# Liaoyongjian1/HC-MVS

Hardware: AMD Instinct MI355X
Metric: PatchMatch Mpix/s (1080p, 8 views, 7x7, 8 iter) (higher is better)
Workload: dtype f32; 1 GPU; batch of 32 independent units per GPU, each 1 ref x 8 src views, 1920x1080, 7x7 taps (adapthalfwin 6), 8 sweeps, it_external 0, full EstimateDepthMap (median + init score + sweeps + end pass); batch=32, exchange=none

## Files before the change

hc-mvs_amd/csrc/est_plan.h:

```cpp
#ifndef HCMVS_EST_PLAN_H
#define HCMVS_EST_PLAN_H
#include <math.h>
#include <stddef.h>
#include <stdint.h>
#include <string.h>
#include "../../include/hcmvs_hip.h"
#include "carve.h"
#include "pm_types.h"
#include "sweep_plan.h"
namespace hcmvs {

inline float fd2r(float d) { return d * (3.14159274101257324f / 180.f); }

inline void mat3_mul(const double* a, const double* b, double* c) {
	for (int i = 0; i < 3; ++i)
		for (int j = 0; j < 3; ++j) {
			double s = 0;
			for (int k = 0; k < 3; ++k) s += a[i * 3 + k] * b[k * 3 + j];
			c[i * 3 + j] = s;
		}
}
inline void mat3_mul_bt(const double* a, const double* b, double* c) {
	for (int i = 0; i < 3; ++i)
		for (int j = 0; j < 3; ++j) {
// ... 94 lines not shown
	k.smoothBonusNormal = (1.f - p.random_smooth_bonus) * 0.96f;
	k.smoothSigmaDepth = -1.f / (2.f * (p.random_smooth_depth * p.random_smooth_depth));
	{ const float r = fd2r(p.random_smooth_normal_deg); k.smoothSigmaNormal = -1.f / (2.f * (r * r)); }
	k.angle1Range = fd2r(p.random_angle1_deg);
	k.angle2Range = fd2r(p.random_angle2_deg);
	k.thConfSmall = p.ncc_threshold_keep * 0.2f;
	k.thConfBig = p.ncc_threshold_keep * 0.4f;
	k.thConfRand = p.ncc_threshold_keep * 0.9f;
	k.thRobust = p.ncc_threshold_keep * 1.2f;
	k.thKeep = p.ncc_threshold_keep;
	k.depthRatio = p.random_depth_ratio;
	k.pfScale = 1.f - p.photometric_flow;
	k.seed = p.seed + seedOffset;
	k.hintIter = est_uses_hint(p, hintOffered) ? p.n_estimation_iters - 1 : -1;
}

inline bool est_view_spreads(bool viewspread, const hcmvs_params& p, bool offersMaps, bool rescaled) {
	return viewspread && p.it_external >= 1 && offersMaps && !rescaled;
}
inline void est_spread_consts(const EstCamera& ref, const EstCamera& s, SpreadView& sv) {
	sv.w = s.w; sv.h = s.h;
	sv.cx = s.K[2]; sv.cy = s.K[5]; sv.ifx = 1.0 / s.K[0]; sv.ify = 1.0 / s.K[4];
	double T[9];
	mat3_mul_bt(ref.R, s.R, T);
	const double dC[3] = {s.C[0] - ref.C[0], s.C[1] - ref.C[1], s.C[2] - ref.C[2]};
	sv.Tz[0] = T[6]; sv.Tz[1] = T[7]; sv.Tz[2] = T[8];
	sv.tz = ref.R[6] * dC[0] + ref.R[7] * dC[1] + ref.R[8] * dC[2];
}

inline SweepItem est_sweep_item(const EstConst& k, int nSweeps, bool prior = false, bool geo = false) {
	return {k.H - 2 * k.border, k.W - 2 * k.border, k.V, k.hintDepth && k.hintIter == nSweeps - 1, k.keep != nullptr, k.spread != nullptr, prior, geo};
}

constexpr uint64_t kEstWindowLimit = 0xFFFF0000ull;
enum EstWindowKind { kEstWindowDirect, kEstWindowSlab, kEstWindowRefused };
struct EstWindow {
	EstWindowKind kind;
	uint64_t base;
	size_t slabBytes;
};
inline EstWindow est_image_window(const uint64_t* addr, const size_t* bytes, int n, uint32_t* off) {
	uint64_t lo = ~(uint64_t)0, hi = 0;
	for (int v = 0; v < n; ++v) {
		if (addr[v] < lo) lo = addr[v];
		if (addr[v] + bytes[v] > hi) hi = addr[v] + bytes[v];
	}
	if (hi - lo < kEstWindowLimit) {
		for (int v = 0; v < n; ++v) off[v] = (uint32_t)(addr[v] - lo);
		return {kEstWindowDirect, lo, 0};
	}
	Carve slab;
	for (int v = 0; v < n; ++v) off[v] = (uint32_t)slab(bytes[v]);
	return {slab.size >= kEstWindowLimit ? kEstWindowRefused : kEstWindowSlab, 0, slab.size};
}

enum PriorBad { kPriorOk = 0, kPriorPara, kPriorSigma, kPriorPhoto2geo };
inline PriorBad est_check_prior_params(const hcmvs_prior_params& pp) {
	if (!(pp.para_prior >= 0.f && pp.para_prior <= 1.f)) return kPriorPara;
	if (!(pp.sigma_prior > 0.f) || !(pp.sigma_prior < INFINITY)) return kPriorSigma;
	if (pp.photo2geo < 0) return kPriorPhoto2geo;
	return kPriorOk;
}
inline bool est_prior_active(bool registered, const hcmvs_prior_params& pp, const hcmvs_params& p) {
	return registered && pp.para_prior > 0.f && p.it_external >= pp.photo2geo;
}
inline void est_prior_consts(const hcmvs_prior_params& pp, int countIter, PriorItem& k) {
// ... 107 lines not shown
```

hc-mvs_amd/csrc/hcmvs_api.cpp:

```cpp
#include "../../include/hcmvs_hip.h"
#include "pm_common.h"
#include "est_plan.h"
#include "fuse_common.h"
#include "pf_chain.h"
#include "filter_plan.h"
#include "fuse_plan.h"
#include "tri_init.h"
#include "cloud_kernels.h"
#include "vis_kernels.h"
#include "mesh_kernels.h"
#include "view_kernels.h"
#include "init_kernels.h"
#include "handoff_kernels.h"
#include "handoff_host.h"
#include "prior_kernels.h"
#include "dev_buf.h"

#include <cmath>
#include <cstdarg>
#include <cstdio>
#include <cstring>
#include <map>
#include <string>
#include <algorithm>
// ... 35 lines not shown

struct hcmvs_ctx final : Reclaimer {
	int device = 0;
	hipStream_t ownStream = nullptr;
	hipStream_t stream = nullptr;
	std::string err;
	std::map<uint32_t, View> views;
	struct Slot {
		explicit Slot(Reclaimer* r) : dn(r), conf(r), tmpDepth(r), progress(r), srcSlab(r) {}
		DevBuf dn, conf, tmpDepth;
		DevBuf progress;
		DevBuf srcSlab;
	};
	std::vector<Slot> slots;
	DevBuf tmpU8{this};
	DevBuf maskStage{this};
	DevBuf sDepth{this}, sNormal{this}, sConf{this};
	DevBuf dViews{this};
	std::vector<DevView> hViews;
	DevBuf dItems{this};
	std::vector<EstConst> hItems;
	DevBuf dSpread{this};
	std::vector<SpreadView> hSpread;
	int viewspread = 0;
	bool haveSpreadStats = false;
	hcmvs_prior_params prior = {0.5f, 0.2f, 2};
	bool havePriorStats = false;
	hcmvs_geo_params geo = {0, 0.25f, 0.15f, 150.f, 160.f, 2, 3.f};
	bool haveGeoStats = false;
	DevBuf dGeo{this};
	std::vector<GeoView> hGeo;
	DevBuf sync{this};
	SweepKnobs knobs;
	DevBuf evals{this};
	Event ev[4];
	int lastSweeps = 0, lastSweepLaunches = 0;
	bool haveStats = false;
	int fuseOrder = 0;
	DevBuf dMaps{this};
	DevBuf counters{this};
	DevBuf fuseScratch{this};
	DevBuf filterStage{this}, filterTab{this}, filterCnt{this};
	DevBuf passScratch{this};
	DevBuf pfState;
	bool errPending = false;
	int nCU = 0;
	PinnedBuf pinned;
	Event upEv[2] = {Event(hipEventDisableTiming), Event(hipEventDisableTiming)};
	DevBuf initBuf{this};
	PinnedBuf initPinned;
	Event initCopied{hipEventDisableTiming};
	bool initInFlight = false;
	Event initEv[2];
	hcmvs_init_stats initStats = {};
	bool haveInitStats = false;
	DevBuf handoffBuf{this};
	PinnedBuf handoffPinned;
	Event handoffEv[2];
	hcmvs_handoff_stats handoffStats = {};
	bool haveHandoffStats = false;
	DevBuf priorGenKept{this};
	PriorGenTrace priorTrace;

	bool reclaim() override {
		if (!pfState.capacity() && !priorGenKept.capacity()) return false;
		(void)hipStreamSynchronize(stream);
// ... 57 lines not shown
	p->random_smooth_bonus = 0.93f;
	p->photometric_flow = 0.f;
	p->seed = 1234;
	p->median_blur = 1;
}

int hcmvs_create(int device, hcmvs_ctx** out) {
	if (!out) return HCMVS_ERR_INVALID;
	*out = nullptr;
	int n = 0;
	if (hipGetDeviceCount(&n) != hipSuccess || n <= 0 || device < 0 || device >= n) return HCMVS_ERR_NO_DEVICE;
	if (hipSetDevice(device) != hipSuccess) return HCMVS_ERR_NO_DEVICE;
	hipDeviceProp_t prop;
	if (hipGetDeviceProperties(&prop, device) != hipSuccess) return HCMVS_ERR_NO_DEVICE;
	if (strncmp(prop.gcnArchName, "gfx950", 6) != 0) return HCMVS_ERR_NO_DEVICE;
	hcmvs_ctx* c = new hcmvs_ctx();
	c->device = device;
	c->nCU = prop.multiProcessorCount;
	if (hipStreamCreateWithFlags(&c->ownStream, hipStreamNonBlocking) != hipSuccess) { hcmvs_destroy(c); return HCMVS_ERR_NO_DEVICE; }
	c->stream = c->ownStream;
	for (Event& e : c->ev)
		if (e.ensure() != hipSuccess) { hcmvs_destroy(c); return HCMVS_ERR_NO_DEVICE; }
	c->hViews.resize((size_t)kMaxBatch * kViewSlotEntries); c->hItems.resize(kMaxBatch); c->hSpread.resize((size_t)kMaxBatch * kMaxViews);
	c->hGeo.resize((size_t)kMaxBatch * kMaxViews);
	if (c->dViews.reserve(sizeof(DevView) * kViewSlotEntries * kMaxBatch, c->stream) != hipSuccess || c->evals.reserve(128, c->stream) != hipSuccess ||
	    c->dSpread.reserve(sizeof(SpreadView) * kMaxViews * kMaxBatch, c->stream) != hipSuccess ||
	    c->dGeo.reserve(sizeof(GeoView) * kMaxViews * kMaxBatch, c->stream) != hipSuccess ||
	    c->dItems.reserve(sizeof(EstConst) * kMaxBatch, c->stream) != hipSuccess || c->sync.reserve(64 + sizeof(int32_t) * 2 * kMaxBatch, c->stream) != hipSuccess) {
		hcmvs_destroy(c);
		return HCMVS_ERR_NO_DEVICE;
	}
	c->knobs = parse_sweep_knobs(getenv("HCMVS_SWEEP_LAG"), getenv("HCMVS_XCD_AFFINITY"), getenv("HCMVS_SWEEP_LAUNCHES"), getenv("HCMVS_SWEEP_SEGMENT"),
	                             getenv("HCMVS_WAVES_PER_ROW"));
	*out = c;
	return HCMVS_OK;
}

void hcmvs_destroy(hcmvs_ctx* c) {
	if (!c) return;
	(void)hipSetDevice(c->device);
	(void)hipStreamSynchronize(c->stream);
	const hipStream_t own = c->ownStream;
	delete c;
	if (own) (void)hipStreamDestroy(own);
}

const char* hcmvs_last_error(const hcmvs_ctx* c) { return c ? c->err.c_str() : "null context"; }

static int check_sweep_error(hcmvs_ctx* c) {
	if (!c->errPending) return HCMVS_OK;
	int32_t flags[2] = {0, 0};
	HIPCHK(c, hipMemcpy(flags, c->sync.get(), sizeof flags, hipMemcpyDeviceToHost));
	c->errPending = false;
	if (flags[1] != 0) return fail(c, HCMVS_ERR_TIMEOUT, "sweep worker timed out waiting for its predecessor row; the maps of the last estimate are incomplete");
	return HCMVS_OK;
}

int hcmvs_set_stream(hcmvs_ctx* c, void* stream) {
	if (!c) return HCMVS_ERR_INVALID;
	c->stream = stream ? (hipStream_t)stream : c->ownStream;
	return HCMVS_OK;
}
int hcmvs_synchronize(hcmvs_ctx* c) {
	if (!c) return HCMVS_ERR_INVALID;
	HIPCHK(c, hipSetDevice(c->device));
	HIPCHK(c, hipStreamSynchronize(c->stream));
// ... 396 lines not shown
		batch.items.push_back(est_sweep_item(k, batch.nSweeps, itemPrior, itemGeo));
		maxRows = std::max(maxRows, batch.items.back().rows);
		spread = spread || k.spread;
		prior = prior || itemPrior;
		geo = geo || itemGeo;
	}
	if (spread) {
		const EstOverlap o = est_spread_overlap(c->hItems.data(), c->hSpread.data(), items, n_items);
		if (o.item >= 0)
			return fail(c, HCMVS_ERR_INVALID, "estimate: the in/out maps of item %d (view %u) overlap the spread maps of source view %u of item %d: "
			            "a launch must not read what it writes (register a copy, or estimate the two images in separate calls)", o.item, items[o.item].ref_id,
			            items[o.other].src_ids[o.view], o.other);
	}
	if (geo) {
		std::vector<char> act((size_t)n_items, 0);
		for (int i = 0; i < n_items; ++i) act[i] = batch.items[i].geo;
		const EstOverlap o = est_geo_overlap(c->hItems.data(), c->hGeo.data(), (const bool*)act.data(), items, n_items);
		if (o.item >= 0)
			return fail(c, HCMVS_ERR_INVALID, "estimate: the in/out maps of item %d (view %u) overlap the maps source view %u of item %d offers to the "
			            "geometric-consistency term: a launch must not read what it writes (register a copy, or estimate the two images in separate calls)",
			            o.item, items[o.item].ref_id, items[o.other].src_ids[o.view], o.other);
	}
	hipStream_t s = c->stream;
	if (geo) HIPCHK(c, hipMemcpyAsync(c->dGeo.get(), c->hGeo.data(), sizeof(GeoView) * kMaxViews * n_items, hipMemcpyHostToDevice, s));
	c->haveGeoStats = geo;
	if (spread) HIPCHK(c, hipMemcpyAsync(c->dSpread.get(), c->hSpread.data(), sizeof(SpreadView) * kMaxViews * n_items, hipMemcpyHostToDevice, s));
	c->haveSpreadStats = spread;
	c->havePriorStats = prior;
	HIPCHK(c, hipMemcpyAsync(c->dViews.get(), c->hViews.data(), sizeof(DevView) * kViewSlotEntries * n_items, hipMemcpyHostToDevice, s));
	HIPCHK(c, hipMemcpyAsync(c->dItems.get(), c->hItems.data(), sizeof(EstConst) * n_items, hipMemcpyHostToDevice, s));
	HIPCHK(c, hipMemsetAsync(c->evals.get(), 0, 128, s));
	HIPCHK(c, hipMemsetAsync(c->sync.get(), 0, 64 + sizeof(int32_t) * 2 * kMaxBatch, s));

	HIPCHK(c, hipEventRecord(c->ev[0].get(), s));
	for (int i = 0; i < n_items; ++i) {
		const EstConst& k = c->hItems[i];
		if (sweepsOnly) { launch_import_state(k, items[i].d_depth, items[i].d_normal, items[i].d_conf, s); continue; }
		const float* depthIn = items[i].d_depth;
		if (k.keep) launch_apply_mask(k.keep, items[i].d_depth, items[i].d_normal, k.W * k.H, s);
		if (p->median_blur) {
			launch_median3(items[i].d_depth, c->slots[i].tmpDepth.get<float>(), k.W, k.H, s);
			depthIn = c->slots[i].tmpDepth.get<float>();
		}
		launch_score_pass(k, depthIn, items[i].d_normal, c->evals.get<unsigned long long>(), s, batch.items[i].prior, batch.items[i].geo);
	}
	HIPCHK(c, hipEventRecord(c->ev[1].get(), s));
	int32_t* sync = c->sync.get<int32_t>();
	const SweepArgs sa{c->dItems.get<EstConst>(), n_items, maxRows, {sync + 16, sync + 16 + kMaxBatch, sync + 1, c->evals.get<unsigned long long>()}, c->knobs.lag, c->knobs.affinity};
	const std::vector<hcmvs::SweepLaunch> plan = hcmvs::plan_sweeps(batch);
	for (const hcmvs::SweepLaunch& l : plan) {
		HIPCHK(c, hipMemsetAsync(sync + 16, 0, sizeof(int32_t) * 2 * kMaxBatch, s));
		for (int i = 0; i < n_items; ++i)
			HIPCHK(c, hipMemsetAsync(c->slots[i].progress.get(), 0, (size_t)batch.items[i].rows * kProgressStride * sizeof(int32_t), s));
		if (!launch_sweep(sa, l, s))
			return fail(c, HCMVS_ERR_INVALID, "estimate: no sweep kernel for %d waves per row, big %d two %d pack %d hint %d mask %d spread %d prior %d geo %d",
			            l.v.nw, l.v.big, l.v.two, l.v.pack, l.v.hint, l.v.mask, l.v.spread, l.v.prior, l.v.geo);
	}
	c->lastSweepLaunches = (int)plan.size();
	HIPCHK(c, hipEventRecord(c->ev[2].get(), s));
	for (int i = 0; i < n_items; ++i)
		launch_end_pass(c->hItems[i], p->it_external == p->n_external_iters - 1 ? 1 : 0, items[i].d_depth, items[i].d_normal, items[i].d_conf, s);
	HIPCHK(c, hipEventRecord(c->ev[3].get(), s));
	HIPCHK(c, hipGetLastError());
	c->lastSweeps = nSweeps;
	c->haveStats = true;
	c->errPending = true;
	return HCMVS_OK;
}

int hcmvs_estimate_batch_device(hcmvs_ctx* c, const hcmvs_batch_item* items, int32_t n_items, const hcmvs_params* p) {
	return estimate_batch(c, items, n_items, p, false, 0, p ? p->n_estimation_iters : 0);
}
int hcmvs_estimate_sweeps_batch_device(hcmvs_ctx* c, const hcmvs_batch_item* items, int32_t n_items, const hcmvs_params* p, int32_t first_sweep,
                                       int32_t n_sweeps) {
	return estimate_batch(c, items, n_items, p, true, first_sweep, n_sweeps);
}

int hcmvs_estimate_device(hcmvs_ctx* c, uint32_t ref_id, const uint32_t* src_ids, int32_t n_src, const hcmvs_params* p,
                          float d_min, float d_max, float* d_depth, float* d_normal, float* d_conf) {
	hcmvs_batch_item it;
	memset(&it, 0, sizeof it);
	it.ref_id = ref_id; it.src_ids = src_ids; it.n_src = n_src; it.d_min = d_min; it.d_max = d_max;
// ... 1288 lines not shown
```

hc-mvs_amd/csrc/pm_common.h:

```cpp
#ifndef HCMVS_PM_COMMON_H
#define HCMVS_PM_COMMON_H

#include <hip/hip_runtime.h>
#include <stdint.h>
#include <utility>
#include "pm_types.h"
#include "sweep_plan.h"

namespace hcmvs {

struct SweepSync {
	int32_t* ticket;
	int32_t* rowsDone;
	int32_t* error;
	unsigned long long* evals;
};

struct SweepArgs {
	const EstConst* dItems;
	int nItems, maxRows;
	SweepSync sync;
	int lag, affinity;
};

void launch_gray_to_u8(const float* gray, uint8_t* out, int n, hipStream_t s);
void launch_bgr_to_u8(const uint8_t* bgr, uint8_t* out, int n, hipStream_t s);
void launch_gradient_map(const uint8_t* g8, uint8_t* gra, int W, int H, hipStream_t s);
void launch_median3(const float* in, float* out, int W, int H, hipStream_t s);
void launch_apply_mask(const uint8_t* keep, float* depth, float* normal, int n, hipStream_t s);
void launch_quads(const float* gray, float4* out, int W, int H, hipStream_t s);
void launch_score_pass(const EstConst& c, const float* depthIn, const float* normalIn, unsigned long long* evals,
                       hipStream_t s, bool prior = false, bool geo = false);
void launch_import_state(const EstConst& c, const float* depthIn, const float* normalIn, const float* confIn, hipStream_t s);
bool launch_sweep(const SweepArgs& a, const SweepLaunch& l, hipStream_t s);
void launch_end_pass(const EstConst& c, int finalPass, float* depth, float* normal, float* conf, hipStream_t s);

}
#endif
```

hc-mvs_amd/csrc/pm_kernels.hip:

```cpp
#include "pm_common.h"
#include "pm_math.h"

#include <float.h>
#include <type_traits>

namespace hcmvs {

#define HC_SQ(x) ((x) * (x))

#ifdef HCMVS_STAMPS
__device__ unsigned long long g_stamps[32];
#define STAMP_DECL unsigned long long st_last = __builtin_amdgcn_s_memtime(), st_acc[16] = {0, 0, 0, 0, 0, 0, 0, 0, 0, 0, 0, 0, 0, 0, 0, 0}; unsigned st_cnt[16] = {0, 0, 0, 0, 0, 0, 0, 0, 0, 0, 0, 0, 0, 0, 0, 0};
#define STAMP(i) { const unsigned long long t_ = __builtin_amdgcn_s_memtime(); st_acc[i] += t_ - st_last; st_last = t_; }
#define STAMP_ARGS , unsigned long long& st_last, unsigned long long (&st_acc)[16], unsigned (&st_cnt)[16]
#define STAMP_PASS , st_last, st_acc, st_cnt
#define STAMP_FLUSH if ((threadIdx.x & 63) == 0 && (threadIdx.x >> 6) == 0) { for (int i_ = 0; i_ < 16; ++i_) atomicAdd(&g_stamps[i_], st_acc[i_]); for (int i_ = 0; i_ < 16; ++i_) atomicAdd(&g_stamps[16 + i_], (unsigned long long)st_cnt[i_]); }
#define SUBMARK(name)
#define BLOCK(name, i) ++st_cnt[i];
#define BLOCKN(name, i, n) st_cnt[i] += (unsigned)(n);
#elif defined(HCMVS_MARK)
#define STAMP_DECL
#define STAMP(i) asm volatile("; HCMARK " #i);
#define SUBMARK(name) asm volatile("; HCMARK " #name);
#define BLOCK(name, i) asm volatile("; HCMARK " #name);
// ... 995 lines not shown
	const int idx = y * c.W + x;
	in.cur = load_dn(&c.dn[idx]);
	in.curConf = load_f(&c.conf[idx]);
	const bool want = in.slot && (!in.isUp || upKnown) && !(in.back > 0 && in.back <= q);
	const int nidx = want ? in.ny * c.W + in.nx : idx;
	in.ndn = load_dn(&c.dn[nidx]);
	in.nconf = load_f(&c.conf[nidx]);
	in.loaded = want;
}
template <int S>
__device__ __forceinline__ void prefetch_up(const EstConst& c, PixIn<S>& in) {
	if (in.isUp && !in.loaded) {
		in.ndn = load_dn(&c.dn[in.ny * c.W + in.nx]);
		in.nconf = load_f(&c.conf[in.ny * c.W + in.nx]);
		in.loaded = true;
	}
}

template <int NW>
__device__ __forceinline__ float share_scores(RowShared<NW>& sh, int& par, int lane, int lo, int hi, float mine) {
	if (NW == 1) return mine;
	if (lane >= lo && lane < hi) sh.sc[par][lane] = mine;
	__syncthreads();
	const float all = sh.sc[par][lane & 31];
	par ^= 1;
	return all;
}

struct SpreadCount { unsigned scored, accepted, dropped, outside; };

template <int S, int NW, bool BIG, bool TWO, bool PACK, bool HINT, bool SPREAD, bool PRIOR = false, bool GEO = false>
__device__ __forceinline__ void process_pixel(const EstConst& c, const LaneCtx<S>& L, const LaneCtx<S>& L1, RowShared<NW>& sh, int& par, int wv,
                                              int x, int y, int q, int iter, const PixIn<S>& in, const Patch<S>& P,
                                              const LdsStore<S>& st, RowPipe<S>& pp, unsigned& evals, unsigned& issued, SpreadCount& spc, const PriorConst& pc, float prior, const GeoPix& gp STAMP_ARGS) {
	static_assert(!PRIOR || !(HINT || SPREAD), "the prior term comes without the hint and without view spread");
	static_assert(!GEO || !(HINT || SPREAD || PRIOR), "the geometric-consistency term comes without the hint, view spread and the prior");
	const int W = c.W, lane = L.lane;
	PixelGeom G;
	pixel_geom(c, x, y, G);

	Close C;
	const int nx = in.nx, ny = in.ny;
	C.d = in.ndn.x; C.n0 = in.ndn.y; C.n1 = in.ndn.z; C.n2 = in.ndn.w; C.conf = in.nconf; C.nx = nx; C.ny = ny;
	if (in.slot && in.back > 0 && in.back <= q) {
		const float* hrec = sh.hist[(q - in.back) & (kHist - 1)];
		C.d = hrec[0]; C.n0 = hrec[1]; C.n1 = hrec[2]; C.n2 = hrec[3]; C.conf = hrec[4];
	}
	C.kd = C.d; C.k0 = C.n0; C.k1 = C.n1; C.k2 = C.n2;
	const bool closeV = in.slot && C.d > 0.f;
	C.closeMask = __ballot(closeV);
	{
		const double z = C.d;
		C.X0 = (float)(((double)nx - c.cx) * z * c.ifx);
		C.X1 = (float)(((double)ny - c.cy) * z * c.ify);
		C.X2 = (float)z;
	}
	const bool elig = closeV && in.sprop && !(C.conf >= c.thKeep);
	C.eligMask = __ballot(elig);
	if (elig) {
		C.kd = interpolate_pixel(c, G, nx, ny, C.d, C.n0, C.n1, C.n2);
		correct_normal(G, C.k0, C.k1, C.k2);
	}
	unsigned long long closeMask = C.closeMask, eligMask = C.eligMask;
	{
		float (*cl)[kMaxSlots] = st.pk->cl;
		if (lane < kMaxSlots) {
			cl[0][lane] = C.X0; cl[1][lane] = C.X1; cl[2][lane] = C.X2;
			cl[3][lane] = C.n0; cl[4][lane] = C.n1; cl[5][lane] = C.n2;
			cl[6][lane] = C.k0; cl[7][lane] = C.k1; cl[8][lane] = C.k2;
		}
	}

	const int idx = y * W + x;
	float conf = in.curConf;
	float depth = in.cur.x, n0 = in.cur.y, n1 = in.cur.z, n2 = in.cur.w;
	init_plane(G, depth, n0, n1, n2);
	STAMP(2)

	enum { PH_PROP, PH_PICK, PH_RAND, PH_REFINE, PH_DONE };
	const int nc = __builtin_popcountll(eligMask);
	int candSlot = 0;
	{
		int i = 0;
		for (unsigned long long mk = eligMask; mk; mk &= mk - 1ull, ++i)
			if (lane == i) candSlot = __builtin_ctzll(mk);
	}
	const float qd = __shfl(C.kd, candSlot, 64), q0 = __shfl(C.k0, candSlot, 64), q1 = __shfl(C.k1, candSlot, 64), q2 = __shfl(C.k2, candSlot, 64);
	const uint32_t rk = rand_key(c.seed, (uint32_t)idx, (uint32_t)c.itExternal * 64u + 1u + (uint32_t)iter);
	const int nR = c.nRandomIters;
	int phase = nc > 0 ? PH_PROP : PH_PICK;
	int cb = 0, t0 = 0;
	unsigned idxScaleRange = 0;
	float scaleRange = 1.f, depthRange = 0.f, p0 = 0.f, p1 = 0.f;
	bool hooked = false, pollTaken = false;
	bool randExit = false;
	for (;;) {
		if (phase == PH_PICK) {
			BLOCK(blk_pick, 0)
			if (!hooked) {
				hooked = true;
				STAMP(5)
				if (pp.pendingPub > 0) {
					asm volatile("s_waitcnt vmcnt(0)" ::: "memory");
					if (lane == 0) __hip_atomic_store(pp.myWord, pp.base + pp.pendingPub, __ATOMIC_RELAXED, HC_SCOPE);
					pp.pendingPub = 0;
				}
				if (pp.r > 0) pp.poll = __hip_atomic_load(pp.upWord, __ATOMIC_RELAXED, HC_SCOPE) - pp.base;
				STAMP(6)
			}
			if (conf <= c.thConfSmall) idxScaleRange = 2;
			else if (conf <= c.thConfBig) idxScaleRange = 1;
			if (conf > c.thConfBig && conf >= c.thConfRand) {
				phase = PH_RAND;
			} else {
				phase = PH_REFINE;
				scaleRange = 1.f / (float)(1u << idxScaleRange);
				depthRange = depth * c.depthRatio;
				p0 = pm_atan2f(n1, n0); p1 = pm_acosf(n2);
				t0 = 0;
			}
		}
		float hd = 0.f, h0 = 0.f, h1 = 0.f, h2 = -1.f, hq0 = 0.f, hq1 = 0.f;
		int hlimit = 63, r0, r1;
		bool hv = false, planeOwn = true;
		if (phase == PH_PROP) {
			BLOCK(blk_gen_prop, 1)
			r0 = cb; r1 = cb + 8 * NW < nc ? cb + 8 * NW : nc;
			hd = qd; h0 = q0; h1 = q1; h2 = q2; hlimit = candSlot;
			hv = lane >= r0 && lane < r1;
		} else if (phase == PH_RAND) {
			BLOCK(blk_gen_rand, 2)
			r0 = 0; r1 = nR; planeOwn = false;
			if (lane < nR) {
				uint32_t rkr = rk;
				asm volatile("" : "+v"(rkr));
				hd = random_depth(c, rand_unit(rkr, 3u * lane));
				random_normal(G, rand_unit(rkr, 3u * lane + 1u), rand_unit(rkr, 3u * lane + 2u), h0, h1, h2);
				hv = true;
			}
		} else {
			BLOCK(blk_gen_refine, 3)
			r0 = t0; r1 = nR;
			if (lane >= t0 && lane < nR) {
				const uint32_t cbase = 64u + 3u * lane;
				hd = depth + (depthRange * scaleRange) * (2.f * rand_unit(rk, cbase) - 1.f);
				if (c.dMin <= hd && hd < c.dMax) {
					hq0 = p0 + (c.angle1Range * scaleRange) * (2.f * rand_unit(rk, cbase + 1u) - 1.f);
					hq1 = p1 + (c.angle2Range * scaleRange) * (2.f * rand_unit(rk, cbase + 2u) - 1.f);
					dir2normal(hq0, hq1, h0, h1, h2);
					hv = !(dot3(h0, h1, h2, G.v0, G.v1, 1.f) >= 0.f);
				}
			}
		}
		const unsigned long long vmask = __ballot(hv);
		const float pkeep = PRIOR && prior > 0.f ? pc.keep : -1.f;
		float PA = 0.f;
		if constexpr (PRIOR) { if (prior > 0.f) PA = prior_addend(pc.sigma, pc.para, prior, hd); }
		STAMP(3)
		const int cnt = r1 - r0, per = (cnt + NW - 1) / NW, lo = r0 + wv * per, hi = (lo + per < r1 ? lo + per : r1);
		float best1 = __builtin_huge_valf(), best2 = __builtin_huge_valf();
		for (int base = lo; base < hi; base += 8) {
			BLOCK(blk_chunk, 4)
			const int g = base + (lane >> 3);
			const int src = g < r1 ? g : r0;
			const float gd = __shfl(hd, src, 64), g0 = __shfl(h0, src, 64), g1 = __shfl(h1, src, 64), g2 = __shfl(h2, src, 64);
			const int glimit = __shfl(hlimit, src, 64);
			const float gp0 = planeOwn ? g0 : G.pn0, gp1 = planeOwn ? g1 : G.pn1, gp2 = planeOwn ? g2 : G.pn2;
			const float gpd = planeOwn ? -gd * dot3(g0, g1, g2, G.v0, G.v1, 1.f) : G.pd;
#if defined(HCMVS_ABL) && HCMVS_ABL == 2
			const float F = 1.f + 0.f * (gd + g0 + g1 + g2 + gp0 + gp1 + gp2 + gpd + (float)glimit);
#else
			BLOCKN(blk_smooth_chunks, 10, closeMask ? (64 - __builtin_clzll(closeMask) + 7) >> 3 : 0)
			const float F = smooth_pass(c, st.pk->cl, closeMask, eligMask, lane, gd, g0, g1, g2, gp0, gp1, gp2, gpd, glimit);
#endif
			const int top = base + 8 < hi ? base + 8 : hi;
			const unsigned long long todo = vmask & ((1ull << top) - 1ull) & ~((1ull << base) - 1ull);
			STAMP(4)
			if (todo) {
				BLOCK(blk_score_chunk, 5)
				score_chunk<S, BIG, PACK, PRIOR, GEO>(c, L, P, st, G.v0, G.v1, F, hd, h0, h1, h2, todo, base, __builtin_ctzll(todo), best1, best2, issued, PA, pkeep, gp);
				if constexpr (TWO) {
					unsigned again = 0;
					score_chunk<S, BIG, PACK, PRIOR, GEO>(c, L1, P, st, G.v0, G.v1, F, hd, h0, h1, h2, todo, base, __builtin_ctzll(todo), best1, best2, again, PA, pkeep, gp);
				}
			}
		}
		const float mine = two_best(c, best1, best2);
		STAMP(7)
		if (hooked && !pollTaken) { pollTaken = true; if (pp.r > 0 && pp.poll > pp.known) pp.known = pp.poll; }
		const float all = share_scores<NW>(sh, par, lane, lo, hi, mine);
		STAMP(8)
		if (phase == PH_PROP) {
			BLOCK(blk_acc_prop, 6)
			for (int i = r0; i < r1; ++i) {
				BLOCK(blk_acc_prop_cand, 7)
				const float nconf = rlf(all, i);
				++evals;
				if (conf > nconf) { conf = nconf; depth = rlf(hd, i); n0 = rlf(h0, i); n1 = rlf(h1, i); n2 = rlf(h2, i); }
				if (i == nc - 1) init_plane(G, rlf(hd, i), rlf(h0, i), rlf(h1, i), rlf(h2, i));
			}
			cb = r1;
			if (cb >= nc) phase = PH_PICK;
		} else if (phase == PH_RAND) {
			BLOCK(blk_acc_rand, 8)
			bool again = false;
			for (int t = 0; t < nR && !again; ++t) {
				const float nconf = rlf(all, t);
				++evals;
				if (conf > nconf) {
					conf = nconf; depth = rlf(hd, t); n0 = rlf(h0, t); n1 = rlf(h1, t); n2 = rlf(h2, t);
					if (conf < c.thConfRand) again = true;
				}
			}
			phase = again ? PH_PICK : PH_DONE;
			if constexpr (SPREAD) randExit = !again;
		} else {
			BLOCK(blk_acc_refine, 9)
			int tnext = nR;
			const unsigned long long range = ((1ull << nR) - 1ull) & ~((1ull << t0) - 1ull);
			const unsigned long long live = vmask & range;
			const unsigned long long better = __ballot(conf > all) & live;
			if (better) {
				const int t = __builtin_ctzll(better);
				evals += (unsigned)__builtin_popcountll(live & ((2ull << t) - 1ull));
				conf = rlf(all, t); depth = rlf(hd, t); n0 = rlf(h0, t); n1 = rlf(h1, t); n2 = rlf(h2, t);
				p0 = rlf(hq0, t); p1 = rlf(hq1, t);
				++idxScaleRange;
				scaleRange = 1.f / (float)(1u << idxScaleRange);
				tnext = t + 1;
			} else {
				evals += (unsigned)__builtin_popcountll(live);
			}
			t0 = tnext;
			if (t0 >= nR) phase = PH_DONE;
		}
// ... 91 lines not shown
				unsigned again = 0;
				score_chunk<S, BIG, PACK>(c, L1, P, st, G.v0, G.v1, F, hd, h0, h1, h2, 1ull, 0, 0, s1, s2, again);
			}
			const float nconf = rlf(two_best(c, s1, s2), 0);
			++evals;
			if (conf > nconf - 0.1f) { conf = nconf; depth = hd; n0 = h0; n1 = h1; n2 = h2; }
		}
	}
	if (hooked && !pollTaken && pp.r > 0 && pp.poll > pp.known) pp.known = pp.poll;
	if (lane == 0) {
		float* hrec = sh.hist[q & (kHist - 1)];
		hrec[0] = depth; hrec[1] = n0; hrec[2] = n1; hrec[3] = n2; hrec[4] = conf;
		if (wv == NW - 1) {
			store_dn(&c.dn[idx], depth, n0, n1, n2);
			store_f(&c.conf[idx], conf);
		}
	}
	if constexpr (NW == 1) {
		pp.pendingPub = q + 1;
	} else if (wv == NW - 1) {
		asm volatile("s_waitcnt vmcnt(0)" ::: "memory");
		if (lane == 0) __hip_atomic_store(pp.myWord, pp.base + q + 1, __ATOMIC_RELAXED, HC_SCOPE);
	}
	STAMP(15)

}


#ifndef HCMVS_OCC
#define HCMVS_OCC 3
#endif
template <int S, int NW, bool BIG, bool TWO = false, bool PACK = false, bool HINT = false, bool MASK = false, bool SPREAD = false, bool PRIOR = false, bool GEO = false>
__global__ __launch_bounds__(64 * NW) __attribute__((amdgpu_waves_per_eu(!BIG ? HCMVS_OCC : 1, !BIG ? HCMVS_OCC : 2))) void sweep_kernel(const EstConst* __restrict__ items, int nItems, int maxRows, SweepSync sy,
                                                        int iter0, int nSweeps, int lag, int affinity, int segLen) {
	__shared__ RowShared<NW> sh;
	__shared__ WavePark<S> park[NW];
	__shared__ float bigTab[BIG ? NW : 1][4][BIG ? kBigSlots : 1];
	const int wv = __builtin_amdgcn_readfirstlane((int)(threadIdx.x >> 6));
	unsigned evals = 0, issued = 0;
	unsigned long long taps = 0;
	SpreadCount spc = {0u, 0u, 0u, 0u};
	GeoPix gp = {nullptr, 0.f, 1.f, 1.f, 0.f, 0.f};
	unsigned evalsGeo = 0, pixelsGeo = 0;
	unsigned evalsPrior = 0, pixelsPrior = 0;
	int par = 0, rot = (int)blockIdx.x;
	STAMP_DECL
	RowPipe<S> pp;
	pp.err = as_global(sy.error);
	for (;;) {
		if (NW > 1) __syncthreads();
		if (threadIdx.x == 0) {
			int item = -1, row = 0;
			const int G = nItems < 8 ? nItems : 8;
			const int home = affinity ? (int)(__builtin_amdgcn_s_getreg(6164) & 7u) % G : 0;
			const int nHome = affinity ? (nItems - home + G - 1) / G : nItems;
			float behind = 2.f;
			if (segLen > 0 && affinity)
				for (int k = 0; k < nItems; ++k) {
					const int nrows_ = items[k].H - 2 * items[k].border;
					const int per_ = nrows_ * ((items[k].W - 2 * items[k].border + segLen - 1) / segLen);
					const int t_ = __hip_atomic_load(as_global(sy.ticket) + k, __ATOMIC_RELAXED, HC_SCOPE);
					if (t_ < per_ * nSweeps) { const float f = (float)t_ / (float)per_; behind = f < behind ? f : behind; }
				}
			for (int pass = 0; pass < 2 && item < 0; ++pass)
				for (int k = 0; k < nItems && item < 0; ++k) {
					int cand;
					if (!affinity) cand = (rot + k) % nItems;
// ... 124 lines not shown
			if (q + 2 < q1) pp.tx2 = uniform_byte(c.gra, y * c.W + x + 2 * dx);
			uint8_t km = 1;
			if constexpr (MASK) km = uniform_byte(c.keep ? c.keep : c.gra, y * c.W + x);
			float prior = 0.f;
			if constexpr (PRIOR) prior = uniform_float(pc.map ? pc.map : c.ref, y * c.W + x);
			STAMP(12)
			Patch<S> P;
			fill_patch<S, BIG>(c, L, x, y, in, P, st);
			STAMP(1)
			if (pp.known < q + 1) {
				pp.known = wait_progress(pp.upWord, pp.base + q + 1, pp.err);
				if (pp.known < 0) {
					pp.fail = true;
					asm volatile("s_waitcnt vmcnt(0)" : "+v"(pp.nI), "+v"(pp.nC) :: "memory");
					break;
				}
				pp.known -= pp.base;
				prefetch_up<S>(c, in);
			}
			asm volatile("s_waitcnt vmcnt(0)" : "+v"(pp.nI), "+v"(pp.nC) :: "memory");
			STAMP(0)
			if (MASK && c.keep && km == 0) {
				if (L.lane == 0) {
					float* hrec = sh.hist[q & (kHist - 1)];
					hrec[0] = in.cur.x; hrec[1] = in.cur.y; hrec[2] = in.cur.z; hrec[3] = in.cur.w; hrec[4] = in.curConf;
					if (wv == NW - 1) __hip_atomic_store(pp.myWord, pp.base + q + 1, __ATOMIC_RELAXED, HC_SCOPE);
				}
				pp.pendingPub = 0;
				continue;
			}
			const unsigned e0 = evals;
			if constexpr (PRIOR) prior = pc.map && prior_usable(prior) ? prior : 0.f;
			if constexpr (GEO) gp = geo_pix(gc, uniform_byte(c.gra, y * c.W + x), x, y);
			process_pixel<S, NW, BIG, TWO, PACK, HINT, SPREAD, PRIOR, GEO>(c, L, L1, sh, par, wv, x, y, q, iter, in, P, st, pp, evals, issued, spc, pc, prior, gp STAMP_PASS);
			taps += (unsigned long long)(evals - e0) * (unsigned)((P.a + 1) * (P.a + 1));
			if constexpr (PRIOR) if (prior > 0.f) { evalsPrior += evals - e0; pixelsPrior += iter == pc.countIter ? 1u : 0u; }
			if constexpr (GEO) if (gp.w > 0.f) { evalsGeo += evals - e0; pixelsGeo += iter == gc.countIter ? 1u : 0u; }
			STAMP(5)
		}
		if (pp.fail) break;
		if (pp.pendingPub > 0) {
			asm volatile("s_waitcnt vmcnt(0)" ::: "memory");
			if ((threadIdx.x & 63) == 0) __hip_atomic_store(pp.myWord, pp.base + pp.pendingPub, __ATOMIC_RELAXED, HC_SCOPE);
			pp.pendingPub = 0;
		}
		if (NW > 1) __syncthreads();
		if (threadIdx.x == 0 && q1 == c.W - 2 * bd) __hip_atomic_fetch_add(as_global(sy.rowsDone) + itemIdx, 1, __ATOMIC_RELAXED, HC_SCOPE);
	}
	STAMP(10)
	STAMP_FLUSH
	if ((threadIdx.x & 63) == 0) {
		if (wv == 0 && evals) { atomicAdd(sy.evals, (unsigned long long)evals); atomicAdd(sy.evals + 2, taps); }
		if (issued) atomicAdd(sy.evals + 1, (unsigned long long)issued);
		if constexpr (SPREAD) if (wv == 0) {
			if (spc.scored) atomicAdd(sy.evals + 4, (unsigned long long)spc.scored);
			if (spc.accepted) atomicAdd(sy.evals + 5, (unsigned long long)spc.accepted);
			if (spc.dropped) atomicAdd(sy.evals + 6, (unsigned long long)spc.dropped);
			if (spc.outside) atomicAdd(sy.evals + 7, (unsigned long long)spc.outside);
		}
		if constexpr (GEO) if (wv == 0) {
			if (evalsGeo) atomicAdd(sy.evals + 10, (unsigned long long)evalsGeo);
			if (pixelsGeo) atomicAdd(sy.evals + 11, (unsigned long long)pixelsGeo);
		}
		if constexpr (PRIOR) if (wv == 0) {
			if (evalsPrior) atomicAdd(sy.evals + 8, (unsigned long long)evalsPrior);
			if (pixelsPrior) atomicAdd(sy.evals + 9, (unsigned long long)pixelsPrior);
		}
	}
}


__global__ void import_kernel(EstConst c, const float* depthIn, const float* normalIn) {
	const int n = c.W * c.H;
	for (int i = blockIdx.x * blockDim.x + threadIdx.x; i < n; i += gridDim.x * blockDim.x) {
		const int x = i % c.W, y = i / c.W;
		const bool inb = x >= c.border && y >= c.border && x < c.W - c.border && y < c.H - c.border;
		if (c.keep && !c.keep[i]) {
			c.dn[i] = make_float4(depthIn[i], 0.f, 0.f, 0.f);
			c.conf[i] = 0.f;
		} else if (inb) {
			c.dn[i] = make_float4(depthIn[i], normalIn[3 * i], normalIn[3 * i + 1], normalIn[3 * i + 2]);
			c.conf[i] = 2.f;
		} else {
			c.dn[i] = make_float4(0.f, 0.f, 0.f, 0.f);
			c.conf[i] = 2.f;
		}
	}
}

__global__ void import_state_kernel(EstConst c, const float* depthIn, const float* normalIn, const float* confIn) {
	const int n = c.W * c.H;
	for (int i = blockIdx.x * blockDim.x + threadIdx.x; i < n; i += gridDim.x * blockDim.x) {
		c.dn[i] = make_float4(depthIn[i], normalIn[3 * i], normalIn[3 * i + 1], normalIn[3 * i + 2]);
		c.conf[i] = confIn[i];
	}
}

template <int S, bool BIG, bool TWO = false, bool MASK = false, bool PRIOR = false, bool GEO = false>
__global__ __launch_bounds__(256) void score_kernel(EstConst c, unsigned long long* evalsOut) {
	LaneCtx<S> L;
	lane_init<S>(c, L);
	__shared__ float stage[4][3][8][8];
	__shared__ float bigTab[BIG ? 4 : 1][4][BIG ? kBigSlots : 1];
	RegStore<S> st;
	st.stage = stage[threadIdx.x >> 6]; st.seg = L.seg;
	st.bw = (float (*)[kBigSlots])(BIG ? &bigTab[BIG ? (threadIdx.x >> 6) : 0][0][0] : nullptr);
	st.put_view(as_global(c.views) + (L.vact ? L.view : 0), L.seg);
	LaneCtx<S> L1 = L;
	RegStore<S> st1 = st;
	if constexpr (TWO) {
		lane_init<S>(c, L1, 64 / S);
		st1.put_view(as_global(c.views) + (L1.vact ? L1.view : 0), L1.seg);
	}
	const int nrows = c.H - 2 * c.border, ncols = c.W - 2 * c.border;
	const int total = nrows * ncols;
	const int wavesPerBlock = blockDim.x >> 6;
	const int gw = blockIdx.x * wavesPerBlock + (threadIdx.x >> 6), nw = gridDim.x * wavesPerBlock;
	unsigned evals = 0, evalsPrior = 0, evalsGeo = 0;
	unsigned long long taps = 0;
// ... 177 lines not shown

void launch_gray_to_u8(const float* gray, uint8_t* out, int n, hipStream_t s) {
	hipLaunchKernelGGL(gray_to_u8_kernel, dim3(2048), dim3(256), 0, s, gray, out, n);
}
void launch_bgr_to_u8(const uint8_t* bgr, uint8_t* out, int n, hipStream_t s) {
	hipLaunchKernelGGL(bgr_to_u8_kernel, dim3(2048), dim3(256), 0, s, bgr, out, n);
}
void launch_gradient_map(const uint8_t* g8, uint8_t* gra, int W, int H, hipStream_t s) {
	hipLaunchKernelGGL(gradient_kernel, dim3((W + 63) / 64, (H + 3) / 4), dim3(64, 4), 0, s, g8, gra, W, H);
}
void launch_quads(const float* gray, float4* out, int W, int H, hipStream_t s) {
	hipLaunchKernelGGL(quad_kernel, dim3((W + 63) / 64, (H + 3) / 4), dim3(64, 4), 0, s, gray, out, W, H);
}
void launch_median3(const float* in, float* out, int W, int H, hipStream_t s) {
	hipLaunchKernelGGL(median3_kernel, dim3((W + 63) / 64, (H + 3) / 4), dim3(64, 4), 0, s, in, out, W, H);
}
void launch_apply_mask(const uint8_t* keep, float* depth, float* normal, int n, hipStream_t s) {
	hipLaunchKernelGGL(apply_mask_kernel, dim3(2048), dim3(256), 0, s, keep, depth, normal, n);
}

template <class K, int N>
struct KernelTable { K at[N]; };
using ScoreKernel = void (*)(EstConst, unsigned long long*);
template <int... I>
static constexpr KernelTable<ScoreKernel, sizeof...(I)> score_table(std::integer_sequence<int, I...>) {
	return {{score_kernel<8, (I & 4) != 0, (I & 2) != 0, (I & 1) != 0, (I & 24) == 8, (I & 16) != 0>...}};
}
static constexpr auto kScoreKernels = score_table(std::make_integer_sequence<int, 24>{});
void launch_score_pass(const EstConst& c, const float* depthIn, const float* normalIn, unsigned long long* evals,
                       hipStream_t s, bool prior, bool geo) {
	hipLaunchKernelGGL(import_kernel, dim3(2048), dim3(256), 0, s, c, depthIn, normalIn);
	hipLaunchKernelGGL(kScoreKernels.at[(geo ? 16 : (prior ? 8 : 0)) | (c.adapthalfwin > kHalfWindow ? 4 : 0) | (c.V > 8 ? 2 : 0) | (c.keep ? 1 : 0)], dim3(4096), dim3(256), 0, s, c, evals);
}
void launch_import_state(const EstConst& c, const float* depthIn, const float* normalIn, const float* confIn, hipStream_t s) {
	hipLaunchKernelGGL(import_state_kernel, dim3(2048), dim3(256), 0, s, c, depthIn, normalIn, confIn);
}

using SweepKernel = void (*)(const EstConst*, int, int, SweepSync, int, int, int, int, int);
constexpr int sweep_variant_index(SweepVariant v) {
	return v.geo << 9 | v.prior << 8 | (v.nw - 1) << 6 | v.big << 5 | v.two << 4 | v.pack << 3 | v.hint << 2 | v.mask << 1 | (int)v.spread;
}
constexpr SweepVariant sweep_variant_at(int i) {
	return {((i >> 6) & 3) + 1, (i & 32) != 0, (i & 16) != 0, (i & 8) != 0, (i & 4) != 0, (i & 2) != 0, (i & 1) != 0, (i & 256) != 0, (i & 512) != 0};
}
template <int I>
static constexpr SweepKernel sweep_instance() {
	constexpr SweepVariant v = sweep_variant_at(I);
	if constexpr (sweep_variant_exists(v)) return sweep_kernel<8, v.nw, v.big, v.two, v.pack, v.hint, v.mask, v.spread, v.prior, v.geo>;
	else return nullptr;
}
template <int... I>
static constexpr KernelTable<SweepKernel, sizeof...(I)> sweep_table(std::integer_sequence<int, I...>) { return {{sweep_instance<I>()...}}; }
static constexpr auto kSweepKernels = sweep_table(std::make_integer_sequence<int, 2 * 2 * 4 * 64>{});

bool launch_sweep(const SweepArgs& a, const SweepLaunch& l, hipStream_t s) {
	const SweepKernel k = sweep_variant_exists(l.v) ? kSweepKernels.at[sweep_variant_index(l.v)] : nullptr;
	if (!k) return false;
	if (l.grid >= 1) hipLaunchKernelGGL(k, dim3(l.grid), dim3(64 * l.v.nw), 0, s, a.dItems, a.nItems, a.maxRows, a.sync, l.first, l.count, a.lag, a.affinity, l.segLen);
	return true;
}

void launch_end_pass(const EstConst& c, int finalPass, float* depth, float* normal, float* conf, hipStream_t s) {
	hipLaunchKernelGGL(end_kernel, dim3(2048), dim3(256), 0, s, c, finalPass, depth, normal, conf);
}

}
```

Baseline: 22.85 Mpix/s.

## Fold initial score pass into first sweep with lazy import of seeded state

Drops the standalone per-item score pass when no hint, spread, prior or geo term is active. A single batched import kernel now seeds depth and normals, replacing out-of-range or back-facing values with random ones. The first sweep scores each pixel's own plane as an extra propagation candidate, so that score becomes its initial cost. This removes a full-image 7x7 multi-view scoring pass and its per-item launches, but makes the first sweep do more work per pixel and changes the order in which costs are evaluated.

Result: no change. 23.02 Mpix/s, median of 6 (+0.7%).

```diff
diff --git a/hc-mvs_amd/csrc/est_plan.h b/hc-mvs_amd/csrc/est_plan.h
--- a/hc-mvs_amd/csrc/est_plan.h
+++ b/hc-mvs_amd/csrc/est_plan.h
@@ -150,6 +150,13 @@
 	return {k.H - 2 * k.border, k.W - 2 * k.border, k.V, k.hintDepth && k.hintIter == nSweeps - 1, k.keep != nullptr, k.spread != nullptr, prior, geo};
 }
 
+inline bool parse_init_score_knob(const char* text) { return !(text && strcmp(text, "pass") == 0); }
+inline bool est_init_score_lazy(bool knobSweep, bool sweepsOnly, const hcmvs_params& p, const std::vector<SweepLaunch>& plan) {
+	if (!knobSweep || sweepsOnly || p.it_external != 0 || plan.empty()) return false;
+	const SweepLaunch& l = plan[0];
+	return l.first == 0 && l.count >= 1 && !(l.v.hint || l.v.spread || l.v.prior || l.v.geo);
+}
+
 constexpr uint64_t kEstWindowLimit = 0xFFFF0000ull;
 enum EstWindowKind { kEstWindowDirect, kEstWindowSlab, kEstWindowRefused };
 struct EstWindow {
diff --git a/hc-mvs_amd/csrc/hcmvs_api.cpp b/hc-mvs_amd/csrc/hcmvs_api.cpp
--- a/hc-mvs_amd/csrc/hcmvs_api.cpp
+++ b/hc-mvs_amd/csrc/hcmvs_api.cpp
@@ -91,6 +91,7 @@
 	std::vector<GeoView> hGeo;
 	DevBuf sync{this};
 	SweepKnobs knobs;
+	bool initScoreSweep = true;
 	DevBuf evals{this};
 	Event ev[4];
 	int lastSweeps = 0, lastSweepLaunches = 0;
@@ -214,6 +215,7 @@
 	}
 	c->knobs = parse_sweep_knobs(getenv("HCMVS_SWEEP_LAG"), getenv("HCMVS_XCD_AFFINITY"), getenv("HCMVS_SWEEP_LAUNCHES"), getenv("HCMVS_SWEEP_SEGMENT"),
 	                             getenv("HCMVS_WAVES_PER_ROW"));
+	c->initScoreSweep = parse_init_score_knob(getenv("HCMVS_INIT_SCORE"));
 	*out = c;
 	return HCMVS_OK;
 }
@@ -676,6 +678,10 @@
 	HIPCHK(c, hipMemsetAsync(c->evals.get(), 0, 128, s));
 	HIPCHK(c, hipMemsetAsync(c->sync.get(), 0, 64 + sizeof(int32_t) * 2 * kMaxBatch, s));
 
+	const std::vector<hcmvs::SweepLaunch> plan = hcmvs::plan_sweeps(batch);
+	const bool lazy = est_init_score_lazy(c->initScoreSweep, sweepsOnly, *p, plan);
+	static_assert(kImportMaxItems == kMaxBatch, "ImportSrc holds an entry per item of a batch");
+	ImportSrc importSrc;
 	HIPCHK(c, hipEventRecord(c->ev[0].get(), s));
 	for (int i = 0; i < n_items; ++i) {
 		const EstConst& k = c->hItems[i];
@@ -686,12 +692,17 @@
 			launch_median3(items[i].d_depth, c->slots[i].tmpDepth.get<float>(), k.W, k.H, s);
 			depthIn = c->slots[i].tmpDepth.get<float>();
 		}
+		if (lazy) { importSrc.depth[i] = depthIn; importSrc.normal[i] = items[i].d_normal; continue; }
 		launch_score_pass(k, depthIn, items[i].d_normal, c->evals.get<unsigned long long>(), s, batch.items[i].prior, batch.items[i].geo);
+	}
+	if (lazy) {
+		for (int i = n_items; i < kMaxBatch; ++i) { importSrc.depth[i] = nullptr; importSrc.normal[i] = nullptr; }
+		launch_lazy_import(c->dItems.get<EstConst>(), n_items, importSrc, s);
 	}
 	HIPCHK(c, hipEventRecord(c->ev[1].get(), s));
 	int32_t* sync = c->sync.get<int32_t>();
-	const SweepArgs sa{c->dItems.get<EstConst>(), n_items, maxRows, {sync + 16, sync + 16 + kMaxBatch, sync + 1, c->evals.get<unsigned long long>()}, c->knobs.lag, c->knobs.affinity};
-	const std::vector<hcmvs::SweepLaunch> plan = hcmvs::plan_sweeps(batch);
+	const SweepArgs sa{c->dItems.get<EstConst>(), n_items, maxRows, {sync + 16, sync + 16 + kMaxBatch, sync + 1, c->evals.get<unsigned long long>()}, c->knobs.lag, c->knobs.affinity,
+	                   lazy ? plan[0].first : -1};
 	for (const hcmvs::SweepLaunch& l : plan) {
 		HIPCHK(c, hipMemsetAsync(sync + 16, 0, sizeof(int32_t) * 2 * kMaxBatch, s));
 		for (int i = 0; i < n_items; ++i)
diff --git a/hc-mvs_amd/csrc/pm_common.h b/hc-mvs_amd/csrc/pm_common.h
--- a/hc-mvs_amd/csrc/pm_common.h
+++ b/hc-mvs_amd/csrc/pm_common.h
@@ -21,6 +21,13 @@
 	int nItems, maxRows;
 	SweepSync sync;
 	int lag, affinity;
+	int lazyIter = -1;
+};
+
+constexpr int kImportMaxItems = 64;
+struct ImportSrc {
+	const float* depth[kImportMaxItems];
+	const float* normal[kImportMaxItems];
 };
 
 void launch_gray_to_u8(const float* gray, uint8_t* out, int n, hipStream_t s);
@@ -31,6 +38,7 @@
 void launch_quads(const float* gray, float4* out, int W, int H, hipStream_t s);
 void launch_score_pass(const EstConst& c, const float* depthIn, const float* normalIn, unsigned long long* evals,
                        hipStream_t s, bool prior = false, bool geo = false);
+void launch_lazy_import(const EstConst* dItems, int nItems, const ImportSrc& src, hipStream_t s);
 void launch_import_state(const EstConst& c, const float* depthIn, const float* normalIn, const float* confIn, hipStream_t s);
 bool launch_sweep(const SweepArgs& a, const SweepLaunch& l, hipStream_t s);
 void launch_end_pass(const EstConst& c, int finalPass, float* depth, float* normal, float* conf, hipStream_t s);
diff --git a/hc-mvs_amd/csrc/pm_kernels.hip b/hc-mvs_amd/csrc/pm_kernels.hip
--- a/hc-mvs_amd/csrc/pm_kernels.hip
+++ b/hc-mvs_amd/csrc/pm_kernels.hip
@@ -1051,9 +1051,10 @@
 template <int S, int NW, bool BIG, bool TWO, bool PACK, bool HINT, bool SPREAD, bool PRIOR = false, bool GEO = false>
 __device__ __forceinline__ void process_pixel(const EstConst& c, const LaneCtx<S>& L, const LaneCtx<S>& L1, RowShared<NW>& sh, int& par, int wv,
                                               int x, int y, int q, int iter, const PixIn<S>& in, const Patch<S>& P,
-                                              const LdsStore<S>& st, RowPipe<S>& pp, unsigned& evals, unsigned& issued, SpreadCount& spc, const PriorConst& pc, float prior, const GeoPix& gp STAMP_ARGS) {
+                                              const LdsStore<S>& st, RowPipe<S>& pp, unsigned& evals, unsigned& issued, SpreadCount& spc, const PriorConst& pc, float prior, const GeoPix& gp, bool lazyIn STAMP_ARGS) {
 	static_assert(!PRIOR || !(HINT || SPREAD), "the prior term comes without the hint and without view spread");
 	static_assert(!GEO || !(HINT || SPREAD || PRIOR), "the geometric-consistency term comes without the hint, view spread and the prior");
+	const bool lazy = !(HINT || SPREAD || PRIOR || GEO) && lazyIn;
 	const int W = c.W, lane = L.lane;
 	PixelGeom G;
 	pixel_geom(c, x, y, G);
@@ -1107,7 +1108,8 @@
 	const float qd = __shfl(C.kd, candSlot, 64), q0 = __shfl(C.k0, candSlot, 64), q1 = __shfl(C.k1, candSlot, 64), q2 = __shfl(C.k2, candSlot, 64);
 	const uint32_t rk = rand_key(c.seed, (uint32_t)idx, (uint32_t)c.itExternal * 64u + 1u + (uint32_t)iter);
 	const int nR = c.nRandomIters;
-	int phase = nc > 0 ? PH_PROP : PH_PICK;
+	const int ncx = nc + (lazy ? 1 : 0);
+	int phase = ncx > 0 ? PH_PROP : PH_PICK;
 	int cb = 0, t0 = 0;
 	unsigned idxScaleRange = 0;
 	float scaleRange = 1.f, depthRange = 0.f, p0 = 0.f, p1 = 0.f;
@@ -1144,8 +1146,9 @@
 		bool hv = false, planeOwn = true;
 		if (phase == PH_PROP) {
 			BLOCK(blk_gen_prop, 1)
-			r0 = cb; r1 = cb + 8 * NW < nc ? cb + 8 * NW : nc;
+			r0 = cb; r1 = cb + 8 * NW < ncx ? cb + 8 * NW : ncx;
 			hd = qd; h0 = q0; h1 = q1; h2 = q2; hlimit = candSlot;
+			if (lazy && lane == nc) { hd = depth; h0 = n0; h1 = n1; h2 = n2; }
 			hv = lane >= r0 && lane < r1;
 		} else if (phase == PH_RAND) {
 			BLOCK(blk_gen_rand, 2)
@@ -1190,7 +1193,8 @@
 			const float F = 1.f + 0.f * (gd + g0 + g1 + g2 + gp0 + gp1 + gp2 + gpd + (float)glimit);
 #else
 			BLOCKN(blk_smooth_chunks, 10, closeMask ? (64 - __builtin_clzll(closeMask) + 7) >> 3 : 0)
-			const float F = smooth_pass(c, st.pk->cl, closeMask, eligMask, lane, gd, g0, g1, g2, gp0, gp1, gp2, gpd, glimit);
+			const float Fs = smooth_pass(c, st.pk->cl, closeMask, eligMask, lane, gd, g0, g1, g2, gp0, gp1, gp2, gpd, glimit);
+			const float F = lazy && phase == PH_PROP && base + (lane >> 3) == nc ? 1.f : Fs;
 #endif
 			const int top = base + 8 < hi ? base + 8 : hi;
 			const unsigned long long todo = vmask & ((1ull << top) - 1ull) & ~((1ull << base) - 1ull);
@@ -1211,7 +1215,10 @@
 		STAMP(8)
 		if (phase == PH_PROP) {
 			BLOCK(blk_acc_prop, 6)
-			for (int i = r0; i < r1; ++i) {
+			if (lazy) { conf = rlf(all, nc); ++evals; }
+			int rc = r1;
+			if constexpr (!(HINT || SPREAD || PRIOR || GEO)) rc = r1 < nc ? r1 : nc;
+			for (int i = r0; i < rc; ++i) {
 				BLOCK(blk_acc_prop_cand, 7)
 				const float nconf = rlf(all, i);
 				++evals;
@@ -1219,7 +1226,7 @@
 				if (i == nc - 1) init_plane(G, rlf(hd, i), rlf(h0, i), rlf(h1, i), rlf(h2, i));
 			}
 			cb = r1;
-			if (cb >= nc) phase = PH_PICK;
+			if (cb >= ncx) phase = PH_PICK;
 		} else if (phase == PH_RAND) {
 			BLOCK(blk_acc_rand, 8)
 			bool again = false;
@@ -1377,7 +1384,7 @@
 #endif
 template <int S, int NW, bool BIG, bool TWO = false, bool PACK = false, bool HINT = false, bool MASK = false, bool SPREAD = false, bool PRIOR = false, bool GEO = false>
 __global__ __launch_bounds__(64 * NW) __attribute__((amdgpu_waves_per_eu(!BIG ? HCMVS_OCC : 1, !BIG ? HCMVS_OCC : 2))) void sweep_kernel(const EstConst* __restrict__ items, int nItems, int maxRows, SweepSync sy,
-                                                        int iter0, int nSweeps, int lag, int affinity, int segLen) {
+                                                        int iter0, int nSweeps, int lag, int affinity, int segLen, int lazyIter) {
 	__shared__ RowShared<NW> sh;
 	__shared__ WavePark<S> park[NW];
 	__shared__ float bigTab[BIG ? NW : 1][4][BIG ? kBigSlots : 1];
@@ -1568,7 +1575,7 @@
 			const unsigned e0 = evals;
 			if constexpr (PRIOR) prior = pc.map && prior_usable(prior) ? prior : 0.f;
 			if constexpr (GEO) gp = geo_pix(gc, uniform_byte(c.gra, y * c.W + x), x, y);
-			process_pixel<S, NW, BIG, TWO, PACK, HINT, SPREAD, PRIOR, GEO>(c, L, L1, sh, par, wv, x, y, q, iter, in, P, st, pp, evals, issued, spc, pc, prior, gp STAMP_PASS);
+			process_pixel<S, NW, BIG, TWO, PACK, HINT, SPREAD, PRIOR, GEO>(c, L, L1, sh, par, wv, x, y, q, iter, in, P, st, pp, evals, issued, spc, pc, prior, gp, iter == lazyIter STAMP_PASS);
 			taps += (unsigned long long)(evals - e0) * (unsigned)((P.a + 1) * (P.a + 1));
 			if constexpr (PRIOR) if (prior > 0.f) { evalsPrior += evals - e0; pixelsPrior += iter == pc.countIter ? 1u : 0u; }
 			if constexpr (GEO) if (gp.w > 0.f) { evalsGeo += evals - e0; pixelsGeo += iter == gc.countIter ? 1u : 0u; }
@@ -1621,6 +1628,39 @@
 			c.dn[i] = make_float4(0.f, 0.f, 0.f, 0.f);
 			c.conf[i] = 2.f;
 		}
+	}
+}
+
+__global__ __launch_bounds__(256) void lazy_import_kernel(const EstConst* __restrict__ items, ImportSrc src) {
+	const EstConst& c = items[blockIdx.y];
+	gcfptr depthIn = (gcfptr)src.depth[blockIdx.y];
+	gcfptr normalIn = (gcfptr)src.normal[blockIdx.y];
+	const HC_GLOBAL uint8_t* keep = as_global(c.keep);
+	const int n = c.W * c.H;
+	const uint32_t stream0 = (uint32_t)c.itExternal * 64u;
+	for (int i = blockIdx.x * blockDim.x + threadIdx.x; i < n; i += gridDim.x * blockDim.x) {
+		const int x = i % c.W, y = i / c.W;
+		const bool inb = x >= c.border && y >= c.border && x < c.W - c.border && y < c.H - c.border;
+		float4 v = make_float4(0.f, 0.f, 0.f, 0.f);
+		float cf = 2.f;
+		if (keep && !keep[i]) {
+			v.x = depthIn[i];
+			cf = 0.f;
+		} else if (inb) {
+			float d = depthIn[i], n0 = normalIn[3 * i], n1 = normalIn[3 * i + 1], n2 = normalIn[3 * i + 2];
+			PixelGeom G;
+			pixel_geom(c, x, y, G);
+			const uint32_t rk = rand_key(c.seed, (uint32_t)i, stream0);
+			if (!(c.dMin <= d && d < c.dMax)) {
+				d = random_depth(c, rand_unit(rk, 0u));
+				random_normal(G, rand_unit(rk, 1u), rand_unit(rk, 2u), n0, n1, n2);
+			} else if (dot3(n0, n1, n2, G.v0, G.v1, 1.f) >= 0.f) {
+				random_normal(G, rand_unit(rk, 1u), rand_unit(rk, 2u), n0, n1, n2);
+			}
+			v = make_float4(d, n0, n1, n2);
+		}
+		c.dn[i] = v;
+		c.conf[i] = cf;
 	}
 }
 
@@ -1864,11 +1904,14 @@
 	hipLaunchKernelGGL(import_kernel, dim3(2048), dim3(256), 0, s, c, depthIn, normalIn);
 	hipLaunchKernelGGL(kScoreKernels.at[(geo ? 16 : (prior ? 8 : 0)) | (c.adapthalfwin > kHalfWindow ? 4 : 0) | (c.V > 8 ? 2 : 0) | (c.keep ? 1 : 0)], dim3(4096), dim3(256), 0, s, c, evals);
 }
+void launch_lazy_import(const EstConst* dItems, int nItems, const ImportSrc& src, hipStream_t s) {
+	hipLaunchKernelGGL(lazy_import_kernel, dim3(nItems > 8 ? 256 : 2048, nItems), dim3(256), 0, s, dItems, src);
+}
 void launch_import_state(const EstConst& c, const float* depthIn, const float* normalIn, const float* confIn, hipStream_t s) {
 	hipLaunchKernelGGL(import_state_kernel, dim3(2048), dim3(256), 0, s, c, depthIn, normalIn, confIn);
 }
 
-using SweepKernel = void (*)(const EstConst*, int, int, SweepSync, int, int, int, int, int);
+using SweepKernel = void (*)(const EstConst*, int, int, SweepSync, int, int, int, int, int, int);
 constexpr int sweep_variant_index(SweepVariant v) {
 	return v.geo << 9 | v.prior << 8 | (v.nw - 1) << 6 | v.big << 5 | v.two << 4 | v.pack << 3 | v.hint << 2 | v.mask << 1 | (int)v.spread;
 }
@@ -1888,7 +1931,7 @@
 bool launch_sweep(const SweepArgs& a, const SweepLaunch& l, hipStream_t s) {
 	const SweepKernel k = sweep_variant_exists(l.v) ? kSweepKernels.at[sweep_variant_index(l.v)] : nullptr;
 	if (!k) return false;
-	if (l.grid >= 1) hipLaunchKernelGGL(k, dim3(l.grid), dim3(64 * l.v.nw), 0, s, a.dItems, a.nItems, a.maxRows, a.sync, l.first, l.count, a.lag, a.affinity, l.segLen);
+	if (l.grid >= 1) hipLaunchKernelGGL(k, dim3(l.grid), dim3(64 * l.v.nw), 0, s, a.dItems, a.nItems, a.maxRows, a.sync, l.first, l.count, a.lag, a.affinity, l.segLen, a.lazyIter);
 	return true;
 }
 
```
